# choyingw/SynergyNet

Measured on AMD Instinct MI355X. Metric: faces/sec (120x120, 68-lmk + 53215-vert), higher is better.
Workload: dtype f32 (fp16x2 split operands, fp32 accumulate)

## Files before the change

synergynet_amd/csrc/fused_block_rm.hip:

```cpp
#include "syn_internal.h"

#include <cstdlib>

namespace syn {

typedef float f32x4 __attribute__((ext_vector_type(4)));
typedef float f32x16 __attribute__((ext_vector_type(16)));
typedef unsigned u32x4 __attribute__((ext_vector_type(4)));
typedef _Float16 f16x8 __attribute__((ext_vector_type(8)));
typedef _Float16 f16x2 __attribute__((ext_vector_type(2)));

namespace {
constexpr int cdivr(int a, int b) { return (a + b - 1) / b; }

__device__ __forceinline__ void split2r(float x0, float x1, unsigned &a, unsigned &b) {
    a = __builtin_bit_cast(unsigned, __builtin_amdgcn_cvt_pkrtz(x0, x1));
    float r0, r1;
    asm("v_fma_mix_f32 %0, %1, -1.0, %2 op_sel_hi:[1,0,0]" : "=v"(r0) : "v"(a), "v"(x0));
    asm("v_fma_mix_f32 %0, %1, -1.0, %2 op_sel:[1,0,0] op_sel_hi:[1,0,0]" : "=v"(r1) : "v"(a), "v"(x1));
    b = __builtin_bit_cast(unsigned, __builtin_amdgcn_cvt_pkrtz(r0, r1));
}
__device__ __forceinline__ f32x16 mfma32r(u32x4 a, u32x4 b, f32x16 c) {
    return __builtin_amdgcn_mfma_f32_32x32x16_f16(__builtin_bit_cast(f16x8, a), __builtin_bit_cast(f16x8, b), c, 0, 0, 0);
}
__device__ __forceinline__ f32x16 mac3r(const u32x4 (&a)[2], const u32x4 (&b)[2], f32x16 c) {
    c = mfma32r(a[1], b[0], c);
    c = mfma32r(a[0], b[1], c);
    c = mfma32r(a[0], b[0], c);
    return c;
}
__device__ __forceinline__ float from_left(float v) {
    return __builtin_bit_cast(float, __builtin_amdgcn_mov_dpp(__builtin_bit_cast(int, v), 0x138 , 0xf, 0xf, true));
}
__device__ __forceinline__ float from_right(float v) {
    return __builtin_bit_cast(float, __builtin_amdgcn_mov_dpp(__builtin_bit_cast(int, v), 0x130 , 0xf, 0xf, true));
}
}

template <int CIN_, int HID_, int COUT_, int H_, int S_, int NF_, bool RES_, int WPE_, int U_, bool LEAN_ = false, int WREG_ = 0, int NBD_ = 1, bool SVC2_ = false>
struct RmCfg {
    static constexpr bool SVC2 = SVC2_;
    static constexpr int NSVW = SVC2_ ? 2 * U_ : U_;
    static constexpr int CIN = CIN_, HID = HID_, COUT = COUT_, H = H_, S = S_, NF = NF_, WPE = WPE_, U = U_;
    static constexpr bool RES = RES_;
    static constexpr bool LEAN = LEAN_;
    static constexpr int WREG = WREG_;
    static constexpr int KS = cdivr(CIN, 16);
    static constexpr int NG = cdivr(HID, 32);
    static constexpr int HIDP = NG * 32;
    static constexpr int NQ = COUT / 8;
    static constexpr int NB = S == 1 ? 1 : 2;
    static constexpr int HO = S == 2 ? H / 2 : H;
    static constexpr int NBD = NBD_, HB = HO / NBD;
    static constexpr int BSTEPS = S == 1 ? cdivr(HB + 2, 3) * 3 : 2 * (HB + 1);
    static_assert(HO % NBD == 0 && (NBD == 1 || !LEAN_), "bands: equal heights; not implemented for the one-slot (LEAN) sums");
    static_assert(!SVC2_ || NBD_ == 1, "two service waves per unit: implemented for the whole-face march");
    static constexpr int NW = NG, NCW = U * NG, NT = (NCW + NSVW) * 64;
    static constexpr int FR = NB * KS;
    static constexpr int XP_DW = FR * 2 * 256, PART_DW = NW * NQ * 256;
    static constexpr int PSLOTS = LEAN ? 1 : 2;
    static constexpr int UNIT_DW = 2 * XP_DW + PSLOTS * PART_DW;
    static constexpr int APL_DW = LEAN ? NG * 2 * 2 * 256 : 0;
    static constexpr int LDS_DW = U * UNIT_DW + 11 * HIDP + 32 + APL_DW;
    static_assert(COUT % 8 == 0 && COUT <= 32, "project tile");
    static_assert(S == 1 || H % 2 == 0, "stride-2 blocks have even input sizes");
    static_assert(S == 1 ? (NF == 1 ? H + 2 <= 32 : 2 * H + 2 <= 32) : (NF == 1 ? H / 2 + 1 <= 32 : H / 2 + 1 <= 16), "one image row per 32-lane block");
    static_assert(!RES || (S == 1 && CIN == COUT), "residual only on stride-1 same-width blocks");
    static_assert(!LEAN || S == 1, "LEAN is implemented for the stride-1 march");
    static_assert(WREG == 0 || (S == 1 && WREG <= 4), "the register-held filter is implemented for the stride-1 march");
    static_assert(S == 2 || H % 3 == 0, "row ring unrolled by 3");
    static_assert(NT <= 1024 && LDS_DW * 4 <= 160 * 1024, "workgroup size / LDS budget");
};

#define SYNR_LAP(i) do { if (PROF) { tn = __builtin_amdgcn_s_memtime(); pt_[i] += tn - tk; tk = tn; } } while (0)
#define SYNR_BARRIER() do { if (PROF) { const unsigned long long tb_ = __builtin_amdgcn_s_memtime(); busy_ += tb_ - tw_; __syncthreads(); tw_ = __builtin_amdgcn_s_memtime(); } else __syncthreads(); } while (0)

template <class C, bool PROF>
__device__ __forceinline__ void rm_block(unsigned *smem, const float *__restrict__ X, const unsigned *__restrict__ Ae3 ,
                           const unsigned *__restrict__ Ap3 , const float *__restrict__ e_shift,
                           const float *__restrict__ Wd , const float *__restrict__ d_shift,
                           const float *__restrict__ p_shift, float *__restrict__ Y, int B, int ub_begin, int ub_end, int ub_step ,
                           const float *__restrict__ scl_e , const float *__restrict__ scl_p,
                           unsigned long long *prof) {
    unsigned long long pt_[7] = {0, 0, 0, 0, 0, 0, 0}, tk = PROF ? __builtin_amdgcn_s_memtime() : 0ull, tn = 0, nsteps = 0;
    const unsigned long long t_begin = tk;
    unsigned long long busy_ = 0, tw_ = tk;
    constexpr int H = C::H, HO = C::HO, NW = C::NW, NT = C::NT;
    const int tid = threadIdx.x, lane = tid & 63;
    const int wave_wg = __builtin_amdgcn_readfirstlane(tid >> 6);
    const bool service = wave_wg >= C::NCW;
    const int uw = service ? (wave_wg - C::NCW) % C::U : wave_wg / NW;
    const bool svc_in = !C::SVC2 || wave_wg - C::NCW < C::U, svc_out = !C::SVC2 || wave_wg - C::NCW >= C::U;
    const int wave = service ? 0 : wave_wg % NW;
    unsigned *Xp = smem + uw * C::UNIT_DW;
    float *Part = reinterpret_cast<float *>(Xp + 2 * C::XP_DW);
    float *Filt = reinterpret_cast<float *>(smem + C::U * C::UNIT_DW);
    float *Esh = Filt + 10 * C::HIDP, *Psh = Esh + C::HIDP;
    unsigned *ApL = reinterpret_cast<unsigned *>(Psh + 32);
    constexpr int DSH = 9 * C::HIDP;
    const int j = lane & 31, h = lane >> 5;
    const int cb = wave * 32 + 4 * h;
    const int nq_live = (C::HID % 32 == 16 && wave == NW - 1) ? 2 : 4;

    int ia, icol[C::NB], oa, ocol;
    if (C::S == 1 && C::NF == 2) {
        ia = j > C::H; icol[0] = (j == 0 || j == C::H + 1) ? -1 : j - 1 - (C::H + 1) * ia; oa = ia; ocol = icol[0];
    } else if (C::S == 1) { ia = 0; icol[0] = j - 1; oa = 0; ocol = j - 1; }
    else if (C::NF == 1) { ia = 0; icol[0] = 2 * j - 1; icol[C::NB - 1] = 2 * j; oa = 0; ocol = j; }
    else { ia = j >> 4; icol[0] = 2 * (j & 15) - 1; icol[C::NB - 1] = 2 * (j & 15); oa = j >> 4; ocol = j & 15; }
    u32x4 ae[C::KS][2], ap[2][2];
    unsigned early_sink = 0;
    if (!service) {
#pragma unroll
        for (int s = 0; s < C::KS; ++s)
#pragma unroll
            for (int p = 0; p < 2; ++p) ae[s][p] = *(const u32x4 *)(Ae3 + ((size_t)(wave * C::KS + s) * 2 + p) * 256 + lane * 4);
        if (!C::LEAN)
#pragma unroll
            for (int s = 0; s < 2; ++s)
#pragma unroll
                for (int p = 0; p < 2; ++p) ap[s][p] = *(const u32x4 *)(Ap3 + ((size_t)(wave * 2 + s) * 2 + p) * 256 + lane * 4);
    } else if (svc_in && ub_begin < ub_end) {
        const int unit = ub_begin + uw, fu = C::NBD > 1 ? unit / C::NBD : unit, r0 = C::NBD > 1 ? (unit - fu * C::NBD) * C::HB : 0;
        const int f_in = fu * C::NF + ia, y0 = C::NBD > 1 ? (C::S == 1 ? r0 - 1 : 2 * (r0 - 1)) : 0;
#pragma unroll
        for (int b = 0; b < C::NB; ++b)
#pragma unroll
            for (int yy = 0; yy < 2; ++yy) {
                const int y = y0 + yy;
                if ((unsigned)icol[b] < (unsigned)H && f_in < B && (unsigned)y < (unsigned)H) {
                    const float *src = X + ((size_t)(f_in * H + y) * H + icol[b]) * C::CIN + 8 * h;
                    asm volatile("global_load_dword %0, %1, off" : "+v"(early_sink) : "v"(src) : "memory");
                }
            }
    }
    const float Se = scl_e[0], c6e = scl_e[1] * (1.0f / 6.0f), inv_sp = scl_p[1] * 6.0f;
    for (int i = tid; i < 9 * C::HIDP; i += NT) { const int c = i % C::HIDP; Filt[i] = c < C::HID ? Wd[(i / C::HIDP) * C::HID + c] : 0.f; }
    for (int i = tid; i < C::HIDP; i += NT) { Filt[DSH + i] = i < C::HID ? d_shift[i] * (1.0f / 6.0f) : 0.f; Esh[i] = i < C::HID ? e_shift[i] * Se : 0.f; }
    if (tid < 32) Psh[tid] = tid < C::COUT ? p_shift[tid] : 0.f;
    if (C::LEAN)
        for (int i = tid; i < C::APL_DW / 4; i += NT) *(u32x4 *)&ApL[4 * i] = *(const u32x4 *)&Ap3[4 * i];

    __syncthreads();
    l2_touch_done(early_sink);

    if (service) {
        __builtin_amdgcn_s_setprio(3);
        for (int ub = ub_begin; ub < ub_end; ub += ub_step) {
            const int unit = ub + uw;
            const int fu = C::NBD > 1 ? unit / C::NBD : unit, r0 = C::NBD > 1 ? (unit - fu * C::NBD) * C::HB : 0;
            const int f_in = fu * C::NF + ia, f_out = fu * C::NF + oa;
            const bool out_ok = (unsigned)ocol < (unsigned)HO && f_out < B;
            f32x4 xr[C::FR][2];
            auto load_row = [&](int y) {
#pragma unroll
                for (int fr = 0; fr < C::FR; ++fr) {
                    const int b = fr / C::KS, sk = fr % C::KS, c0 = 16 * sk + 8 * h;
                    xr[fr][0] = (f32x4){0.f, 0.f, 0.f, 0.f}; xr[fr][1] = xr[fr][0];
                    if (c0 + 8 <= C::CIN && (unsigned)icol[b] < (unsigned)H && f_in < B && (C::NBD == 1 || (unsigned)y < (unsigned)H)) {
                        const float *src = X + ((size_t)(f_in * H + y) * H + icol[b]) * C::CIN + c0;
                        xr[fr][0] = *(const f32x4 *)src; xr[fr][1] = *(const f32x4 *)(src + 4);
                    }
                }
            };
            auto store_row = [&](int slot) {
#pragma unroll
                for (int fr = 0; fr < C::FR; ++fr) {
                    u32x4 pc[2];
#pragma unroll
                    for (int t = 0; t < 2; ++t) {
                        unsigned a0, b0, a1, b1;
                        split2r(xr[fr][t][0], xr[fr][t][1], a0, b0);
                        split2r(xr[fr][t][2], xr[fr][t][3], a1, b1);
                        pc[0][2 * t] = a0; pc[0][2 * t + 1] = a1; pc[1][2 * t] = b0; pc[1][2 * t + 1] = b1;
                    }
                    unsigned *dst = Xp + (size_t)slot * C::XP_DW + fr * 512 + lane * 4;
#pragma unroll
                    for (int p = 0; p < 2; ++p) *(u32x4 *)(dst + p * 256) = pc[p];
                }
            };
            f32x4 res[C::RES ? C::NQ : 1];
            auto load_res = [&](int yo) {
                if (C::RES) {
#pragma unroll
                    for (int q = 0; q < C::NQ; ++q) {
                        res[q] = (f32x4){0.f, 0.f, 0.f, 0.f};
                        if (out_ok && yo >= 0 && yo < HO) res[q] = *(const f32x4 *)(X + ((size_t)(f_out * H + yo) * H + ocol) * C::CIN + 8 * q + 4 * h);
                    }
                }
            };
            auto reduce_row = [&](int yo, int pslot) {
#pragma unroll
                for (int q = 0; q < C::NQ; ++q) {
                    const float *src = Part + (size_t)pslot * C::PART_DW + q * 256 + lane * 4;
                    f32x4 v = *(const f32x4 *)src;
#pragma unroll
                    for (int w = 1; w < NW; ++w) v += *(const f32x4 *)(src + (size_t)w * C::NQ * 256);
                    v = v * inv_sp + *(const f32x4 *)&Psh[8 * q + 4 * h];
                    if (C::RES) v += res[q];
                    if (out_ok) *(f32x4 *)(Y + ((size_t)(f_out * HO + yo) * HO + ocol) * C::COUT + 8 * q + 4 * h) = v;
                }
            };
            if (C::NBD > 1) {
                constexpr int NS = C::BSTEPS, HB = C::HB;
                const int gy0 = C::S == 1 ? r0 - 1 : 2 * (r0 - 1);
                load_row(gy0);
                store_row(0);
                load_row(gy0 + 1);
                SYNR_BARRIER();
                for (int k = 0; k < NS; ++k) {
                    if (C::S == 1) {
                        if (k >= 3 && k < HB + 3) reduce_row(r0 + k - 3, (k - 1) & 1);
                        if (k >= 2) load_res(r0 + k - 2);
                    } else {
                        if (!(k & 1) && k >= 4) reduce_row(r0 + (k >> 1) - 2, ((k >> 1) - 1) & 1);
                    }
                    if (k + 1 < NS) store_row((k + 1) & 1);
                    if (k + 2 < NS) load_row(gy0 + k + 2);
                    SYNR_BARRIER();
                }
                if (C::S == 2) reduce_row(r0 + HB - 1, HB & 1);
                else if (NS == HB + 2) reduce_row(r0 + HB - 1, (NS - 1) & 1);
                continue;
            }
            if (svc_in) { load_row(0); store_row(0); load_row(1); }
            SYNR_BARRIER();
            if (C::S == 1) {
                if (svc_out) load_res(0);
                constexpr int PM = C::PSLOTS - 1;
                for (int y = 0; y < H; ++y) {
                    if (svc_out && y >= 2) reduce_row(y - 2, y & PM);
                    if (C::LEAN) SYNR_BARRIER();
                    if (svc_out) load_res(y - 1);
                    if (svc_in && y + 1 < H) store_row((y + 1) & 1);
                    if (svc_in && y + 2 < H) load_row(y + 2);
                    SYNR_BARRIER();
                }
                if (svc_out) reduce_row(H - 2, (H - 2) & PM);
                if (C::LEAN) SYNR_BARRIER();
                if (svc_out) load_res(H - 1);
                SYNR_BARRIER();
                if (svc_out) reduce_row(H - 1, (H - 1) & PM);
            } else {
                for (int y = 0; y < H; ++y) {
                    if (svc_out && !(y & 1) && y >= 2) reduce_row((y >> 1) - 1, ((y >> 1) - 1) & 1);
                    if (svc_in && y + 1 < H) store_row((y + 1) & 1);
                    if (svc_in && y + 2 < H) load_row(y + 2);
                    SYNR_BARRIER();
                }
                if (svc_out) reduce_row(HO - 1, (HO - 1) & 1);
            }
        }
        if (PROF && lane == 0) atomicAdd(&prof[8 + wave_wg], busy_);
        return;
    }

    f32x4 wreg[C::WREG > 0 ? C::WREG : 1][9], wbase[C::WREG > 0 ? C::WREG : 1];
#pragma unroll
    for (int q = 0; q < C::WREG; ++q) {
#pragma unroll
        for (int k = 0; k < 9; ++k) wreg[q][k] = *(const f32x4 *)(Filt + cb + 8 * q + k * C::HIDP);
        wbase[q] = *(const f32x4 *)(Filt + cb + 8 * q + DSH);
    }
    for (int ub = ub_begin; ub < ub_end; ub += ub_step) {
        const int unit = ub + uw;
        const int fu = C::NBD > 1 ? unit / C::NBD : unit, r0 = C::NBD > 1 ? (unit - fu * C::NBD) * C::HB : 0;
        const int f_in = fu * C::NF + ia;
        float ehi[C::NB];
        float ehs[C::NB];
#pragma unroll
        for (int b = 0; b < C::NB; ++b) ehs[b] = ehi[b] = ((unsigned)icol[b] < (unsigned)H && f_in < B) ? c6e : 0.0f;
        auto row_ceiling = [&](int gy) {
#pragma unroll
            for (int b = 0; b < C::NB; ++b) ehs[b] = (unsigned)gy < (unsigned)H ? ehi[b] : 0.0f;
        };

        auto expand = [&](int slot, int b, f32x16 &e, int cbo) {
#pragma unroll
            for (int q = 0; q < 4; ++q) {
                const f32x4 sh = *(const f32x4 *)&Esh[cbo + 8 * q];
#pragma unroll
                for (int t = 0; t < 4; ++t) e[4 * q + t] = sh[t];
            }
#pragma unroll
            for (int s = 0; s < C::KS; ++s) {
                u32x4 xb[2];
                const unsigned *src = Xp + (size_t)slot * C::XP_DW + (b * C::KS + s) * 512 + lane * 4;
#pragma unroll
                for (int p = 0; p < 2; ++p) xb[p] = *(const u32x4 *)(src + p * 256);
                e = mac3r(ae[s], xb, e);
            }
#pragma unroll
            for (int r = 0; r < 16; ++r) e[r] = __builtin_amdgcn_fmed3f(e[r] * ehs[b], 0.0f, 1.0f);
        };
        auto finalize = [&](f32x16 &d, int pslot, bool raw = false) {
            f32x16 acc;
#pragma unroll
            for (int r = 0; r < 16; ++r) acc[r] = 0.f;
#pragma unroll
            for (int s = 0; s < 2; ++s) {
                if (2 * s >= nq_live) break;
                u32x4 db[2];
#pragma unroll
                for (int t = 0; t < 4; ++t) {
                    float v0 = d[8 * s + 2 * t], v1 = d[8 * s + 2 * t + 1];
                    if (raw) { v0 = __builtin_amdgcn_fmed3f(v0, 0.0f, 1.0f); v1 = __builtin_amdgcn_fmed3f(v1, 0.0f, 1.0f); }
                    unsigned ha, hb;
                    split2r(v0, v1, ha, hb);
                    db[0][t] = ha; db[1][t] = hb;
                }
                if (C::LEAN) {
                    u32x4 apl[2];
#pragma unroll
                    for (int p = 0; p < 2; ++p) apl[p] = *(const u32x4 *)(ApL + ((size_t)(wave * 2 + s) * 2 + p) * 256 + lane * 4);
                    acc = mac3r(apl, db, acc);
                } else {
                    acc = mac3r(ap[s], db, acc);
                }
            }
            float *dst = Part + (size_t)pslot * C::PART_DW + (size_t)wave * C::NQ * 256 + lane * 4;
#pragma unroll
            for (int q = 0; q < C::NQ; ++q) *(f32x4 *)(dst + q * 256) = (f32x4){acc[4 * q], acc[4 * q + 1], acc[4 * q + 2], acc[4 * q + 3]};
        };
        auto taps3 = [&](f32x16 &d, int q, const float *wq, int ky, const f32x4 &l4, const f32x4 &c4, const f32x4 &r4, bool init, bool last = false) {
            const f32x4 w0 = *(const f32x4 *)(wq + (3 * ky + 0) * C::HIDP), w1 = *(const f32x4 *)(wq + (3 * ky + 1) * C::HIDP),
                        w2 = *(const f32x4 *)(wq + (3 * ky + 2) * C::HIDP);
            f32x4 base;
            if (init) base = *(const f32x4 *)(wq + DSH);
#pragma unroll
            for (int t = 0; t < 4; ++t) {
                const float b0 = init ? base[t] : d[4 * q + t];
                const float v = __builtin_fmaf(r4[t], w2[t], __builtin_fmaf(c4[t], w1[t], __builtin_fmaf(l4[t], w0[t], b0)));
                d[4 * q + t] = last ? __builtin_amdgcn_fmed3f(v, 0.0f, 1.0f) : v;
            }
#pragma unroll
            for (int t = 0; t < 4; ++t) asm volatile("" : "+v"(d[4 * q + t]));
        };
        auto taps3r = [&](f32x16 &d, int q, const f32x4 *wr, const f32x4 &base, int ky, const f32x4 &l4, const f32x4 &c4, const f32x4 &r4, bool init, bool last = false) {
#pragma unroll
            for (int t = 0; t < 4; ++t) {
                const float b0 = init ? base[t] : d[4 * q + t];
                const float v = __builtin_fmaf(r4[t], wr[3 * ky + 2][t], __builtin_fmaf(c4[t], wr[3 * ky + 1][t], __builtin_fmaf(l4[t], wr[3 * ky][t], b0)));
                d[4 * q + t] = last ? __builtin_amdgcn_fmed3f(v, 0.0f, 1.0f) : v;
            }
#pragma unroll
            for (int t = 0; t < 4; ++t) asm volatile("" : "+v"(d[4 * q + t]));
        };
        auto taps2 = [&](f32x16 &d, int q, const float *wq, int ta, int tb, const f32x4 &c4, const f32x4 &r4, bool init) {
            const f32x4 wa = *(const f32x4 *)(wq + ta * C::HIDP), wb = *(const f32x4 *)(wq + tb * C::HIDP);
            f32x4 base;
            if (init) base = *(const f32x4 *)(wq + DSH);
#pragma unroll
            for (int t = 0; t < 4; ++t) d[4 * q + t] = __builtin_fmaf(r4[t], wb[t], __builtin_fmaf(c4[t], wa[t], init ? base[t] : d[4 * q + t]));
#pragma unroll
            for (int t = 0; t < 4; ++t) asm volatile("" : "+v"(d[4 * q + t]));
        };
        auto taps1 = [&](f32x16 &d, int q, const float *wq, int ta, const f32x16 &e, bool last = false) {
            const f32x4 wa = *(const f32x4 *)(wq + ta * C::HIDP);
#pragma unroll
            for (int t = 0; t < 4; ++t) {
                const float v = __builtin_fmaf(e[4 * q + t], wa[t], d[4 * q + t]);
                d[4 * q + t] = last ? __builtin_amdgcn_fmed3f(v, 0.0f, 1.0f) : v;
            }
#pragma unroll
            for (int t = 0; t < 4; ++t) asm volatile("" : "+v"(d[4 * q + t]));
        };
        auto opaque_cb = [&]() { int c = cb; asm volatile("" : "+v"(c)); return c; };

        SYNR_BARRIER();

        if (C::S == 1) {
            f32x16 d0, d1, d2;
            {
                const int cbo = opaque_cb();
#pragma unroll
                for (int q = 0; q < 4; ++q) {
                    const f32x4 sh = *(const f32x4 *)(Filt + cbo + 8 * q + DSH);
#pragma unroll
                    for (int t = 0; t < 4; ++t) { d0[4 * q + t] = sh[t]; d1[4 * q + t] = 0.f; d2[4 * q + t] = 0.f; }
                }
            }
            auto step = [&](int xslot, bool fin, int pslot, f32x16 &dm, f32x16 &dc, f32x16 &dn) {
                SYNR_LAP(5);
                const int cbo = opaque_cb();
                f32x16 e;
                expand(xslot, 0, e, cbo);
                SYNR_LAP(1);
#pragma unroll
                for (int q = 0; q < 4; ++q) {
                    if (q >= nq_live) break;
                    f32x4 c4, l4, r4;
#pragma unroll
                    for (int t = 0; t < 4; ++t) { c4[t] = e[4 * q + t]; l4[t] = from_left(c4[t]); r4[t] = from_right(c4[t]); }
                    const float *wq = Filt + cbo + 8 * q;
                    if (q < C::WREG) {
                        taps3r(dn, q, wreg[q < C::WREG ? q : 0], wbase[q < C::WREG ? q : 0], 0, l4, c4, r4, true);
                        taps3r(dc, q, wreg[q < C::WREG ? q : 0], wbase[q < C::WREG ? q : 0], 1, l4, c4, r4, false);
                        taps3r(dm, q, wreg[q < C::WREG ? q : 0], wbase[q < C::WREG ? q : 0], 2, l4, c4, r4, false, true);
                    } else {
                        taps3(dn, q, wq, 0, l4, c4, r4, true);
                        taps3(dc, q, wq, 1, l4, c4, r4, false);
                        taps3(dm, q, wq, 2, l4, c4, r4, false, true);
                    }
                    __builtin_amdgcn_sched_barrier(0);
                }
                SYNR_LAP(3);
                if (C::LEAN) SYNR_BARRIER();
                if (fin) finalize(dm, pslot);
                SYNR_LAP(4);
                SYNR_BARRIER();
                nsteps += 1;
            };
            if (C::NBD > 1) {
                auto bstep = [&](int k, f32x16 &dm, f32x16 &dc, f32x16 &dn) {
                    row_ceiling(r0 - 1 + k);
                    step(k & 1, k >= 2 && k < C::HB + 2, k & 1, dm, dc, dn);
                };
                for (int k = 0; k < C::BSTEPS; k += 3) {
                    bstep(k, d2, d0, d1);
                    bstep(k + 1, d0, d1, d2);
                    bstep(k + 2, d1, d2, d0);
                }
            } else {
                for (int y = 0; y < H; y += 3) {
                    step(y & 1, y >= 1, (y - 1) & (C::PSLOTS - 1), d2, d0, d1);
                    step((y + 1) & 1, true, y & (C::PSLOTS - 1), d0, d1, d2);
                    step((y + 2) & 1, true, (y + 1) & (C::PSLOTS - 1), d1, d2, d0);
                }
                if (C::LEAN) SYNR_BARRIER();
                finalize(d2, (H - 1) & (C::PSLOTS - 1), true);
                SYNR_BARRIER();
            }
        } else {
            f32x16 dcur, dnext;
            {
                const int cbo = opaque_cb();
#pragma unroll
                for (int q = 0; q < 4; ++q) {
                    const f32x4 sh = *(const f32x4 *)(Filt + cbo + 8 * q + DSH);
#pragma unroll
                    for (int t = 0; t < 4; ++t) { dcur[4 * q + t] = sh[t]; dnext[4 * q + t] = 0.f; }
                }
            }
            const int np = C::NBD > 1 ? C::HB + 1 : HO, p0 = C::NBD > 1 ? r0 - 1 : 0;
            for (int lp = 0; lp < np; ++lp) {
                const int yo = p0 + lp;
                {
                    if (C::NBD > 1) row_ceiling(2 * yo);
                    SYNR_LAP(5);
                    const int cbo = opaque_cb();
                    f32x16 e;
                    expand(0, 0, e, cbo);
#pragma unroll
                    for (int q = 0; q < 4; ++q) {
                        if (q >= nq_live) break;
                        f32x4 c4, r4;
#pragma unroll
                        for (int t = 0; t < 4; ++t) { c4[t] = e[4 * q + t]; r4[t] = from_right(c4[t]); }
                        taps2(dcur, q, Filt + cbo + 8 * q, 3, 5, c4, r4, false);
                        __builtin_amdgcn_sched_barrier(0);
                    }
                    expand(0, 1, e, cbo);
#pragma unroll
                    for (int q = 0; q < 4; ++q) {
                        if (q >= nq_live) break;
                        taps1(dcur, q, Filt + cbo + 8 * q, 4, e);
                        __builtin_amdgcn_sched_barrier(0);
                    }
                    SYNR_LAP(3);
                    SYNR_BARRIER();
                    nsteps += 1;
                }
                {
                    if (C::NBD > 1) row_ceiling(2 * yo + 1);
                    SYNR_LAP(5);
                    const int cbo = opaque_cb();
                    f32x16 e;
                    expand(1, 0, e, cbo);
#pragma unroll
                    for (int q = 0; q < 4; ++q) {
                        if (q >= nq_live) break;
                        f32x4 c4, r4;
#pragma unroll
                        for (int t = 0; t < 4; ++t) { c4[t] = e[4 * q + t]; r4[t] = from_right(c4[t]); }
                        taps2(dcur, q, Filt + cbo + 8 * q, 6, 8, c4, r4, false);
                        taps2(dnext, q, Filt + cbo + 8 * q, 0, 2, c4, r4, true);
                        __builtin_amdgcn_sched_barrier(0);
                    }
                    expand(1, 1, e, cbo);
#pragma unroll
                    for (int q = 0; q < 4; ++q) {
                        if (q >= nq_live) break;
                        taps1(dcur, q, Filt + cbo + 8 * q, 7, e, true);
                        taps1(dnext, q, Filt + cbo + 8 * q, 1, e);
                        __builtin_amdgcn_sched_barrier(0);
                    }
                    SYNR_LAP(3);
                    if (C::NBD == 1 || lp >= 1) finalize(dcur, lp & 1);
                    SYNR_LAP(4);
                    dcur = dnext;
                    SYNR_BARRIER();
                    nsteps += 1;
                }
            }
        }
    }
    if (PROF && lane == 0) atomicAdd(&prof[8 + wave_wg], busy_);
    if (PROF && tid == 0) {
        pt_[6] = __builtin_amdgcn_s_memtime() - t_begin;
        for (int i = 0; i < 7; ++i) atomicAdd(&prof[i], pt_[i]);
        atomicAdd(&prof[7], nsteps);
    }
}

template <class C, bool PROF = false>
__global__ __launch_bounds__(C::NT) __attribute__((amdgpu_waves_per_eu(C::WPE, C::WPE)))
void fused_block_rm_kernel(const float *__restrict__ X, const unsigned *__restrict__ Ae3, const unsigned *__restrict__ Ap3, const float *__restrict__ e_shift,
                           const float *__restrict__ Wd, const float *__restrict__ d_shift, const float *__restrict__ p_shift, float *__restrict__ Y, int B,
                           int n_units, const float *__restrict__ scl_e, const float *__restrict__ scl_p, unsigned long long *prof = nullptr) {
    __shared__ __attribute__((aligned(16))) unsigned smem[C::LDS_DW];
    rm_block<C, PROF>(smem, X, Ae3, Ap3, e_shift, Wd, d_shift, p_shift, Y, B, blockIdx.x * C::U, n_units, gridDim.x * C::U, scl_e, scl_p, prof);
}

struct RmStageArgs {
    const float *X; const unsigned *Ae3, *Ap3; const float *e_shift, *Wd, *d_shift, *p_shift; float *Y; const float *scl_e, *scl_p;
};
template <class CA, class CB>
__global__ __launch_bounds__(CA::NT) __attribute__((amdgpu_waves_per_eu(CA::WPE, CA::WPE)))
void fused_pair_rm_kernel(RmStageArgs a, RmStageArgs b, int B) {
    static_assert(CA::NT == CB::NT && CA::WPE == CB::WPE && CA::NBD == 1 && CB::NBD == 1, "one workgroup shape for both blocks; whole-face marches");
    constexpr int FA = CA::U * CA::NF, FB = CB::U * CB::NF, FG = FA > FB ? FA : FB;
    static_assert(FG % FA == 0 && FG % FB == 0, "a group is whole rounds of both blocks");
    __shared__ __attribute__((aligned(16))) unsigned smem[CA::LDS_DW > CB::LDS_DW ? CA::LDS_DW : CB::LDS_DW];
    const int nua = (B + CA::NF - 1) / CA::NF, nub = (B + CB::NF - 1) / CB::NF;
    {
        const int gq = blockIdx.x;
        const int ua = gq * (FG / CA::NF), ub = gq * (FG / CB::NF);
        rm_block<CA, false>(smem, a.X, a.Ae3, a.Ap3, a.e_shift, a.Wd, a.d_shift, a.p_shift, a.Y, B, ua, ua + FG / CA::NF < nua ? ua + FG / CA::NF : nua, CA::U,
                            a.scl_e, a.scl_p, nullptr);
        __builtin_amdgcn_fence(__ATOMIC_RELEASE, "workgroup");
        __syncthreads();
        __builtin_amdgcn_fence(__ATOMIC_ACQUIRE, "workgroup");
        rm_block<CB, false>(smem, b.X, b.Ae3, b.Ap3, b.e_shift, b.Wd, b.d_shift, b.p_shift, b.Y, B, ub, ub + FG / CB::NF < nub ? ub + FG / CB::NF : nub, CB::U,
                            b.scl_e, b.scl_p, nullptr);
    }
}

template <class C>
static void launch_rm(const FusedBlockArgs &a, int B, hipStream_t s, int wgs_per_cu) {
    const int n_units = (B + C::NF - 1) / C::NF * C::NBD;
    const int cap = 256 * wgs_per_cu, wgs = (n_units + C::U - 1) / C::U;
    const int grid = wgs < cap ? wgs : cap;
    if (a.prof)
        fused_block_rm_kernel<C, true><<<grid, C::NT, 0, s>>>(a.X, a.Arm_e, a.Arm_p, a.e_shift, a.Wd, a.d_shift, a.p_shift, a.Y, B, n_units, a.scl_e, a.scl_p, a.prof);
    else
        fused_block_rm_kernel<C><<<grid, C::NT, 0, s>>>(a.X, a.Arm_e, a.Arm_p, a.e_shift, a.Wd, a.d_shift, a.p_shift, a.Y, B, n_units, a.scl_e, a.scl_p);
}

template <int U> using R2 = RmCfg< 16,  96,  24, 60, 2, 1, false, (U == 4 ? 4 : 3), U>;
template <int U> using R3 = RmCfg< 24, 144,  24, 30, 1, 1, true,  3, U, false, 1>;
template <int U> using R4 = RmCfg< 24, 144,  32, 30, 2, 2, false, 3, U>;
template <int U> using R5 = RmCfg< 32, 192,  32, 15, 1, 2, true,  4, U, true, 0, 1, true>;
template <int U, int NBD> using R2b = RmCfg< 16,  96,  24, 60, 2, 1, false, 3, U, false, 0, NBD>;
template <int U, int NBD> using R3b = RmCfg< 24, 144,  24, 30, 1, 1, true,  3, U, false, 1, NBD>;
constexpr int kBand2Min = 40, kBand3Min = 96;

template <class CA, class CB>
static void launch_pair(const FusedBlockArgs &a, const FusedBlockArgs &b, int B, hipStream_t s) {
    constexpr int FA = CA::U * CA::NF, FB = CB::U * CB::NF, FG = FA > FB ? FA : FB;
    const int n_groups = (B + FG - 1) / FG;
    fused_pair_rm_kernel<CA, CB><<<n_groups, CA::NT, 0, s>>>(RmStageArgs{a.X, a.Arm_e, a.Arm_p, a.e_shift, a.Wd, a.d_shift, a.p_shift, a.Y, a.scl_e, a.scl_p},
                                                        RmStageArgs{b.X, b.Arm_e, b.Arm_p, b.e_shift, b.Wd, b.d_shift, b.p_shift, b.Y, b.scl_e, b.scl_p}, B);
}
bool launch_fused_pair_rm(int first, const FusedBlockArgs &a, const FusedBlockArgs &b, int B, hipStream_t s) {
    static const bool on56 = test_knob("rm_pair56", 1) != 0, on34 = test_knob("rm_pair34", 1) != 0;
    if (B < 513 || a.prof || b.prof) return false;
    if (!a.Arm_e || !a.Arm_p || !a.scl_e || !a.scl_p || !b.Arm_e || !b.Arm_p || !b.scl_e || !b.scl_p) return false;
    if (first == 5 && on56) { launch_pair<R5<2>, R5<2>>(a, b, B, s); return true; }
    if (first == 3 && on34 && (B + 3) / 4 <= 256) { launch_pair<R3<2>, R4<2>>(a, b, B, s); return true; }
    return false;
}

bool launch_fused_block_rm(int feature, const FusedBlockArgs &a, int B, hipStream_t s) {
    if (!a.Arm_e || !a.Arm_p || !a.scl_e || !a.scl_p) return false;
    static const bool bands2 = test_knob("rm_band2", 1) != 0, bands3 = test_knob("rm_band3", 1) != 0;
    switch (feature) {
        case 2:
            if (B >= 513) { launch_rm<R2<4>>(a, B, s, 1); return true; }
            if (B >= 352) { launch_rm<R2<2>>(a, B, s, 1); return true; }
            if (bands2 && B >= kBand2Min) { launch_rm<R2b<1, 6>>(a, B, s, 3); return true; }
            return false;
        case 3:
            if (B >= 448) { launch_rm<R3<2>>(a, B, s, 1); return true; }
            if (B >= 200) { launch_rm<R3<1>>(a, B, s, 1); return true; }
            if (bands3 && B >= kBand3Min) { launch_rm<R3b<2, 3>>(a, B, s, 1); return true; }
            return false;
        case 4:
            if (B >= 513) { launch_rm<R4<2>>(a, B, s, 1); return true; }
            if (B >= 480) { launch_rm<R4<1>>(a, B, s, 1); return true; }
            return false;
        case 5:
        case 6:
            if (B >= 513) { launch_rm<R5<2>>(a, B, s, 1); return true; }
            return false;
        default: return false;
    }
}

}
```

Measured before the change: 1.024 million.

## Use buffer loads/stores with OOB clamping in service waves and restructure row marches

Service waves now load and store through buffer resources whose range covers only the unit's faces. Out-of-range rows and columns get an out-of-bounds offset and return zero, which replaces per-element branches and 64-bit address math. The row marches are rewritten: first and last steps are peeled, the residual and input rows can be double-buffered when there are two service waves, and the stride-2 reduction is split across two barrier halves. Compute waves can also keep the expand shift vector in registers (EREG, enabled for R2/R4/R2b), and the depthwise accumulator swap is replaced by ping-pong unrolling, at the cost of more registers and code size.

```diff
diff --git a/synergynet_amd/csrc/fused_block_rm.hip b/synergynet_amd/csrc/fused_block_rm.hip
--- a/synergynet_amd/csrc/fused_block_rm.hip
+++ b/synergynet_amd/csrc/fused_block_rm.hip
@@ -37,8 +37,9 @@
 }
 }
 
-template <int CIN_, int HID_, int COUT_, int H_, int S_, int NF_, bool RES_, int WPE_, int U_, bool LEAN_ = false, int WREG_ = 0, int NBD_ = 1, bool SVC2_ = false>
+template <int CIN_, int HID_, int COUT_, int H_, int S_, int NF_, bool RES_, int WPE_, int U_, bool LEAN_ = false, int WREG_ = 0, int NBD_ = 1, bool SVC2_ = false, bool EREG_ = false>
 struct RmCfg {
+    static constexpr bool EREG = EREG_;
     static constexpr bool SVC2 = SVC2_;
     static constexpr int NSVW = SVC2_ ? 2 * U_ : U_;
     static constexpr int CIN = CIN_, HID = HID_, COUT = COUT_, H = H_, S = S_, NF = NF_, WPE = WPE_, U = U_;
@@ -90,7 +91,7 @@
     const int wave_wg = __builtin_amdgcn_readfirstlane(tid >> 6);
     const bool service = wave_wg >= C::NCW;
     const int uw = service ? (wave_wg - C::NCW) % C::U : wave_wg / NW;
-    const bool svc_in = !C::SVC2 || wave_wg - C::NCW < C::U, svc_out = !C::SVC2 || wave_wg - C::NCW >= C::U;
+    const bool svc_in = !C::SVC2 || wave_wg - C::NCW < C::U;
     const int wave = service ? 0 : wave_wg % NW;
     unsigned *Xp = smem + uw * C::UNIT_DW;
     float *Part = reinterpret_cast<float *>(Xp + 2 * C::XP_DW);
@@ -146,32 +147,46 @@
 
     if (service) {
         __builtin_amdgcn_s_setprio(3);
+        constexpr unsigned OOB = 0x40000000u;
+        constexpr unsigned IN_ROW_B = H * C::CIN * 4, IN_FACE_B = H * IN_ROW_B, OUT_ROW_B = HO * C::COUT * 4, OUT_FACE_B = HO * OUT_ROW_B;
+        static_assert((unsigned long long)C::NF * IN_FACE_B < OOB && (unsigned long long)C::NF * OUT_FACE_B < OOB, "a unit's faces fit the offset range");
+        constexpr int XB = C::SVC2 ? 2 : 1;
+        constexpr int RB = C::SVC2 && C::RES ? 2 : 1;
+        constexpr int QH = C::S == 2 ? (C::NQ + 1) / 2 : C::NQ;
+        unsigned xo[C::FR];
+#pragma unroll
+        for (int fr = 0; fr < C::FR; ++fr) {
+            const int b = fr / C::KS, sk = fr % C::KS, c0 = 16 * sk + 8 * h;
+            xo[fr] = (c0 + 8 <= C::CIN && (unsigned)icol[b] < (unsigned)H) ? (unsigned)((ia * H * H + icol[b]) * C::CIN + c0) * 4u : OOB;
+        }
+        const unsigned reso = (unsigned)ocol < (unsigned)HO ? (unsigned)((oa * H * H + ocol) * C::CIN + 4 * h) * 4u : OOB;
+        const unsigned outo = (unsigned)ocol < (unsigned)HO ? (unsigned)((oa * HO * HO + ocol) * C::COUT + 4 * h) * 4u : OOB;
+        auto units = [&](const bool in, const bool out) {
         for (int ub = ub_begin; ub < ub_end; ub += ub_step) {
             const int unit = ub + uw;
             const int fu = C::NBD > 1 ? unit / C::NBD : unit, r0 = C::NBD > 1 ? (unit - fu * C::NBD) * C::HB : 0;
-            const int f_in = fu * C::NF + ia, f_out = fu * C::NF + oa;
-            const bool out_ok = (unsigned)ocol < (unsigned)HO && f_out < B;
-            f32x4 xr[C::FR][2];
-            auto load_row = [&](int y) {
+            const long long f0 = (long long)fu * C::NF;
+            const int nf = (long long)B - f0 >= C::NF ? C::NF : ((long long)B > f0 ? (int)((long long)B - f0) : 0);
+            const __amdgpu_buffer_rsrc_t rsx = __builtin_amdgcn_make_buffer_rsrc(const_cast<float *>(X) + (size_t)f0 * (IN_FACE_B / 4), 0, nf * (int)IN_FACE_B, 0x00027000);
+            const __amdgpu_buffer_rsrc_t rsy = __builtin_amdgcn_make_buffer_rsrc(Y + (size_t)f0 * (OUT_FACE_B / 4), 0, nf * (int)OUT_FACE_B, 0x00027000);
+            f32x4 xr[XB][C::FR][2];
+            auto load_row = [&](int y, bool ok, int xb) {
+                const unsigned rowo = (ok && (unsigned)y < (unsigned)H) ? (unsigned)y * IN_ROW_B : OOB;
 #pragma unroll
                 for (int fr = 0; fr < C::FR; ++fr) {
-                    const int b = fr / C::KS, sk = fr % C::KS, c0 = 16 * sk + 8 * h;
-                    xr[fr][0] = (f32x4){0.f, 0.f, 0.f, 0.f}; xr[fr][1] = xr[fr][0];
-                    if (c0 + 8 <= C::CIN && (unsigned)icol[b] < (unsigned)H && f_in < B && (C::NBD == 1 || (unsigned)y < (unsigned)H)) {
-                        const float *src = X + ((size_t)(f_in * H + y) * H + icol[b]) * C::CIN + c0;
-                        xr[fr][0] = *(const f32x4 *)src; xr[fr][1] = *(const f32x4 *)(src + 4);
-                    }
+                    xr[xb][fr][0] = __builtin_bit_cast(f32x4, __builtin_amdgcn_raw_buffer_load_b128(rsx, xo[fr] + rowo, 0, 0));
+                    xr[xb][fr][1] = __builtin_bit_cast(f32x4, __builtin_amdgcn_raw_buffer_load_b128(rsx, xo[fr] + rowo, 16, 0));
                 }
             };
-            auto store_row = [&](int slot) {
+            auto store_row = [&](int slot, int xb) {
 #pragma unroll
                 for (int fr = 0; fr < C::FR; ++fr) {
                     u32x4 pc[2];
 #pragma unroll
                     for (int t = 0; t < 2; ++t) {
                         unsigned a0, b0, a1, b1;
-                        split2r(xr[fr][t][0], xr[fr][t][1], a0, b0);
-                        split2r(xr[fr][t][2], xr[fr][t][3], a1, b1);
+                        split2r(xr[xb][fr][t][0], xr[xb][fr][t][1], a0, b0);
+                        split2r(xr[xb][fr][t][2], xr[xb][fr][t][3], a1, b1);
                         pc[0][2 * t] = a0; pc[0][2 * t + 1] = a1; pc[1][2 * t] = b0; pc[1][2 * t + 1] = b1;
                     }
                     unsigned *dst = Xp + (size_t)slot * C::XP_DW + fr * 512 + lane * 4;
@@ -179,78 +194,117 @@
                     for (int p = 0; p < 2; ++p) *(u32x4 *)(dst + p * 256) = pc[p];
                 }
             };
-            f32x4 res[C::RES ? C::NQ : 1];
-            auto load_res = [&](int yo) {
+            f32x4 res[C::RES ? RB : 1][C::RES ? C::NQ : 1];
+            auto load_res = [&](int yo, bool ok, int rb) {
                 if (C::RES) {
-#pragma unroll
-                    for (int q = 0; q < C::NQ; ++q) {
-                        res[q] = (f32x4){0.f, 0.f, 0.f, 0.f};
-                        if (out_ok && yo >= 0 && yo < HO) res[q] = *(const f32x4 *)(X + ((size_t)(f_out * H + yo) * H + ocol) * C::CIN + 8 * q + 4 * h);
-                    }
+                    const unsigned rowo = (ok && (unsigned)yo < (unsigned)HO) ? (unsigned)yo * IN_ROW_B : OOB;
+#pragma unroll
+                    for (int q = 0; q < C::NQ; ++q) res[rb][q] = __builtin_bit_cast(f32x4, __builtin_amdgcn_raw_buffer_load_b128(rsx, reso + rowo, 32 * q, 0));
                 }
             };
-            auto reduce_row = [&](int yo, int pslot) {
-#pragma unroll
-                for (int q = 0; q < C::NQ; ++q) {
+            auto reduce_row = [&](int yo, int pslot, bool ok, int rb, int q0, int q1) {
+                const unsigned rowo = ok ? (unsigned)yo * OUT_ROW_B : OOB;
+#pragma unroll
+                for (int q = q0; q < q1; ++q) {
                     const float *src = Part + (size_t)pslot * C::PART_DW + q * 256 + lane * 4;
                     f32x4 v = *(const f32x4 *)src;
 #pragma unroll
                     for (int w = 1; w < NW; ++w) v += *(const f32x4 *)(src + (size_t)w * C::NQ * 256);
                     v = v * inv_sp + *(const f32x4 *)&Psh[8 * q + 4 * h];
-                    if (C::RES) v += res[q];
-                    if (out_ok) *(f32x4 *)(Y + ((size_t)(f_out * HO + yo) * HO + ocol) * C::COUT + 8 * q + 4 * h) = v;
-                }
+                    if (C::RES) v += res[rb][q];
+                    __builtin_amdgcn_raw_buffer_store_b128(__builtin_bit_cast(u32x4, v), rsy, outo + rowo, 32 * q, 0);
+                }
+            };
+            auto pair_steps = [&](int g, int yo, int pslot, bool ok, bool st0, bool ld0, bool st1, bool ld1) {
+                if (st0) store_row(1, 0);
+                if (ld0) load_row(g + 2, true, 0);
+                reduce_row(yo, pslot, ok, 0, 0, QH);
+                SYNR_BARRIER();
+                if (st1) store_row(0, 0);
+                if (ld1) load_row(g + 3, true, 0);
+                reduce_row(yo, pslot, ok, 0, QH, C::NQ);
+                SYNR_BARRIER();
             };
             if (C::NBD > 1) {
                 constexpr int NS = C::BSTEPS, HB = C::HB;
                 const int gy0 = C::S == 1 ? r0 - 1 : 2 * (r0 - 1);
-                load_row(gy0);
-                store_row(0);
-                load_row(gy0 + 1);
+                load_row(gy0, true, 0);
+                store_row(0, 0);
+                load_row(gy0 + 1, true, 0);
+                if (C::S == 1) {
+                    static_assert(C::S == 2 || NS >= 4, "band march: a peeled first step, two last steps");
+                    load_res(0, false, 0);
+                    SYNR_BARRIER();
+                    auto bstep = [&](int k, int in, bool last) {
+                        if (in >= 1) store_row((k + 1) & 1, 0);
+                        if (in >= 2) load_row(gy0 + k + 2, true, 0);
+                        reduce_row(r0 + k - 3, (k - 1) & 1, k >= 3 && k < HB + 3, 0, 0, C::NQ);
+                        if (!last || NS == HB + 2) load_res(r0 + k - 2, k >= 2, 0);
+                        SYNR_BARRIER();
+                    };
+                    bstep(0, 2, false);
+#pragma unroll 1
+                    for (int k = 1; k < NS - 2; ++k) bstep(k, 2, false);
+                    bstep(NS - 2, 1, false);
+                    bstep(NS - 1, 0, true);
+                    if (NS == HB + 2) reduce_row(r0 + HB - 1, (NS - 1) & 1, true, 0, 0, C::NQ);
+                } else {
+                    SYNR_BARRIER();
+                    pair_steps(gy0, 0, 0, false, true, true, true, true);
+#pragma unroll 1
+                    for (int k = 2; k < NS - 2; k += 2) pair_steps(gy0 + k, r0 + (k >> 1) - 2, ((k >> 1) - 1) & 1, k >= 4, true, true, true, true);
+                    pair_steps(gy0 + NS - 2, r0 + (NS >> 1) - 3, ((NS >> 1) - 2) & 1, NS >= 6, true, false, false, false);
+                    reduce_row(r0 + HB - 1, HB & 1, true, 0, 0, C::NQ);
+                }
+                continue;
+            }
+            if (C::S == 1) {
+                constexpr int PM = C::PSLOTS - 1;
+                constexpr int LF = H - 2 - XB;
+                constexpr int LE = RB + (LF + 1 - RB) / RB * RB;
+                static_assert(LF >= RB && (XB == 1 || RB == 2), "row march: peeled first steps; one parity for the row and the residual buffers");
+                auto step = [&](const bool in, const bool out, int y, int xb, int rb, bool st, bool ld) {
+                    if (in && st) store_row((y + 1) & 1, xb);
+                    if (in && ld) load_row(y + 1 + XB, true, xb);
+                    if (out && RB == 2) load_res(y - 1, true, rb ^ 1);
+                    if (out) reduce_row(y - 2, y & PM, y >= 2, rb, 0, C::NQ);
+                    if (C::LEAN) SYNR_BARRIER();
+                    if (out && RB == 1) load_res(y - 1, true, 0);
+                    SYNR_BARRIER();
+                };
+                auto march = [&](const bool in, const bool out) {
+                    if (in) {
+                        load_row(0, true, 0); store_row(0, 0); load_row(1, true, XB - 1);
+                        if (XB == 2) load_row(2, true, 0);
+                    }
+                    if (out) load_res(0, false, 0);
+                    SYNR_BARRIER();
+#pragma unroll
+                    for (int r = 0; r < RB; ++r) step(in, out, r, (r + 1) & (XB - 1), r, true, true);
+#pragma unroll 1
+                    for (int y = RB; y < LE; y += RB)
+#pragma unroll
+                        for (int r = 0; r < RB; ++r) step(in, out, y + r, (r + 1) & (XB - 1), r, true, true);
+#pragma unroll
+                    for (int y = LE; y <= H; ++y) step(in, out, y, (y + 1) & (XB - 1), y & (RB - 1), y <= H - 2, y <= LF);
+                    if (out) reduce_row(H - 1, (H - 1) & PM, true, (H + 1) & (RB - 1), 0, C::NQ);
+                };
+                march(in, out);
+            } else {
+                static_assert(C::S == 1 || (!C::SVC2 && H >= 6), "stride-2 march: one service wave; a peeled first and last pair");
+                load_row(0, true, 0); store_row(0, 0); load_row(1, true, 0);
                 SYNR_BARRIER();
-                for (int k = 0; k < NS; ++k) {
-                    if (C::S == 1) {
-                        if (k >= 3 && k < HB + 3) reduce_row(r0 + k - 3, (k - 1) & 1);
-                        if (k >= 2) load_res(r0 + k - 2);
-                    } else {
-                        if (!(k & 1) && k >= 4) reduce_row(r0 + (k >> 1) - 2, ((k >> 1) - 1) & 1);
-                    }
-                    if (k + 1 < NS) store_row((k + 1) & 1);
-                    if (k + 2 < NS) load_row(gy0 + k + 2);
-                    SYNR_BARRIER();
-                }
-                if (C::S == 2) reduce_row(r0 + HB - 1, HB & 1);
-                else if (NS == HB + 2) reduce_row(r0 + HB - 1, (NS - 1) & 1);
-                continue;
-            }
-            if (svc_in) { load_row(0); store_row(0); load_row(1); }
-            SYNR_BARRIER();
-            if (C::S == 1) {
-                if (svc_out) load_res(0);
-                constexpr int PM = C::PSLOTS - 1;
-                for (int y = 0; y < H; ++y) {
-                    if (svc_out && y >= 2) reduce_row(y - 2, y & PM);
-                    if (C::LEAN) SYNR_BARRIER();
-                    if (svc_out) load_res(y - 1);
-                    if (svc_in && y + 1 < H) store_row((y + 1) & 1);
-                    if (svc_in && y + 2 < H) load_row(y + 2);
-                    SYNR_BARRIER();
-                }
-                if (svc_out) reduce_row(H - 2, (H - 2) & PM);
-                if (C::LEAN) SYNR_BARRIER();
-                if (svc_out) load_res(H - 1);
-                SYNR_BARRIER();
-                if (svc_out) reduce_row(H - 1, (H - 1) & PM);
-            } else {
-                for (int y = 0; y < H; ++y) {
-                    if (svc_out && !(y & 1) && y >= 2) reduce_row((y >> 1) - 1, ((y >> 1) - 1) & 1);
-                    if (svc_in && y + 1 < H) store_row((y + 1) & 1);
-                    if (svc_in && y + 2 < H) load_row(y + 2);
-                    SYNR_BARRIER();
-                }
-                if (svc_out) reduce_row(HO - 1, (HO - 1) & 1);
+                pair_steps(0, 0, 0, false, true, true, true, true);
+#pragma unroll 1
+                for (int y = 2; y < H - 2; y += 2) pair_steps(y, (y >> 1) - 1, ((y >> 1) - 1) & 1, true, true, true, true, true);
+                pair_steps(H - 2, (H >> 1) - 2, ((H >> 1) - 2) & 1, true, true, false, false, false);
+                reduce_row(HO - 1, (HO - 1) & 1, true, 0, 0, C::NQ);
             }
         }
+        };
+        if (!C::SVC2) units(true, true);
+        else if (svc_in) units(true, false);
+        else units(false, true);
         if (PROF && lane == 0) atomicAdd(&prof[8 + wave_wg], busy_);
         return;
     }
@@ -262,6 +316,14 @@
         for (int k = 0; k < 9; ++k) wreg[q][k] = *(const f32x4 *)(Filt + cb + 8 * q + k * C::HIDP);
         wbase[q] = *(const f32x4 *)(Filt + cb + 8 * q + DSH);
     }
+    f32x16 esh_r;
+    if (C::EREG)
+#pragma unroll
+        for (int q = 0; q < 4; ++q) {
+            const f32x4 sh = *(const f32x4 *)&Esh[cb + 8 * q];
+#pragma unroll
+            for (int t = 0; t < 4; ++t) esh_r[4 * q + t] = sh[t];
+        }
     for (int ub = ub_begin; ub < ub_end; ub += ub_step) {
         const int unit = ub + uw;
         const int fu = C::NBD > 1 ? unit / C::NBD : unit, r0 = C::NBD > 1 ? (unit - fu * C::NBD) * C::HB : 0;
@@ -276,12 +338,14 @@
         };
 
         auto expand = [&](int slot, int b, f32x16 &e, int cbo) {
-#pragma unroll
-            for (int q = 0; q < 4; ++q) {
-                const f32x4 sh = *(const f32x4 *)&Esh[cbo + 8 * q];
-#pragma unroll
-                for (int t = 0; t < 4; ++t) e[4 * q + t] = sh[t];
-            }
+            if (C::EREG) e = esh_r;
+            else
+#pragma unroll
+                for (int q = 0; q < 4; ++q) {
+                    const f32x4 sh = *(const f32x4 *)&Esh[cbo + 8 * q];
+#pragma unroll
+                    for (int t = 0; t < 4; ++t) e[4 * q + t] = sh[t];
+                }
 #pragma unroll
             for (int s = 0; s < C::KS; ++s) {
                 u32x4 xb[2];
@@ -432,18 +496,18 @@
                 SYNR_BARRIER();
             }
         } else {
-            f32x16 dcur, dnext;
+            f32x16 dA, dB;
             {
                 const int cbo = opaque_cb();
 #pragma unroll
                 for (int q = 0; q < 4; ++q) {
                     const f32x4 sh = *(const f32x4 *)(Filt + cbo + 8 * q + DSH);
 #pragma unroll
-                    for (int t = 0; t < 4; ++t) { dcur[4 * q + t] = sh[t]; dnext[4 * q + t] = 0.f; }
-                }
-            }
-            const int np = C::NBD > 1 ? C::HB + 1 : HO, p0 = C::NBD > 1 ? r0 - 1 : 0;
-            for (int lp = 0; lp < np; ++lp) {
+                    for (int t = 0; t < 4; ++t) { dA[4 * q + t] = sh[t]; dB[4 * q + t] = 0.f; }
+                }
+            }
+            const int p0 = C::NBD > 1 ? r0 - 1 : 0;
+            auto pair = [&](int lp, f32x16 &dcur, f32x16 &dnext) {
                 const int yo = p0 + lp;
                 {
                     if (C::NBD > 1) row_ceiling(2 * yo);
@@ -498,11 +562,13 @@
                     SYNR_LAP(3);
                     if (C::NBD == 1 || lp >= 1) finalize(dcur, lp & 1);
                     SYNR_LAP(4);
-                    dcur = dnext;
                     SYNR_BARRIER();
                     nsteps += 1;
                 }
-            }
+            };
+            constexpr int NP = C::NBD > 1 ? C::HB + 1 : HO;
+            for (int lp = 0; lp + 1 < NP; lp += 2) { pair(lp, dA, dB); pair(lp + 1, dB, dA); }
+            if (NP & 1) pair(NP - 1, dA, dB);
         }
     }
     if (PROF && lane == 0) atomicAdd(&prof[8 + wave_wg], busy_);
@@ -557,11 +623,11 @@
         fused_block_rm_kernel<C><<<grid, C::NT, 0, s>>>(a.X, a.Arm_e, a.Arm_p, a.e_shift, a.Wd, a.d_shift, a.p_shift, a.Y, B, n_units, a.scl_e, a.scl_p);
 }
 
-template <int U> using R2 = RmCfg< 16,  96,  24, 60, 2, 1, false, (U == 4 ? 4 : 3), U>;
+template <int U> using R2 = RmCfg< 16,  96,  24, 60, 2, 1, false, (U == 4 ? 4 : 3), U, false, 0, 1, false, true>;
 template <int U> using R3 = RmCfg< 24, 144,  24, 30, 1, 1, true,  3, U, false, 1>;
-template <int U> using R4 = RmCfg< 24, 144,  32, 30, 2, 2, false, 3, U>;
+template <int U> using R4 = RmCfg< 24, 144,  32, 30, 2, 2, false, 3, U, false, 0, 1, false, true>;
 template <int U> using R5 = RmCfg< 32, 192,  32, 15, 1, 2, true,  4, U, true, 0, 1, true>;
-template <int U, int NBD> using R2b = RmCfg< 16,  96,  24, 60, 2, 1, false, 3, U, false, 0, NBD>;
+template <int U, int NBD> using R2b = RmCfg< 16,  96,  24, 60, 2, 1, false, 3, U, false, 0, NBD, false, true>;
 template <int U, int NBD> using R3b = RmCfg< 24, 144,  24, 30, 1, 1, true,  3, U, false, 1, NBD>;
 constexpr int kBand2Min = 40, kBand3Min = 96;
 
```

Result: no change. 1.024 million, median of 4 (+0.1%).
